# aerius-labs/paillier-halo2

Measured on AMD Instinct MI355X. Metric: Paillier-encrypt proofs/s (2048-bit n, k=17); MSM achieved HBM GB/s vs peak, higher is better.
Workload: dtype u32 limbs (29-bit reduced radix, 254-bit modular integers), u64 limbs (4096-bit integers)

## Files before the change

paillier_halo2_amd/csrc/pz_quotient.hip:

```cpp
#include "fp29.cuh"
#include "pz_internal.h"

static inline Fr fp_one_host() {
    static const uint64_t ONE[4] = {0xac96341c4ffffffbULL, 0x36fc76959f60cd29ULL, 0x666ea36f7879462eULL, 0x0e0a77c19a07df2fULL};
    Fr r;
    memcpy(r.v, ONE, 32);
    return r;
}
static inline Fr fr_from_u64(const uint64_t x[4]) {
    Fr r;
    memcpy(r.v, x, 32);
    return r;
}

typedef F29<FrTag> Fr29;
__device__ __forceinline__ Fr29 fr29_c261(const Fr& c) { return f29_to_261(f29_from_fp(c)); }
__device__ __forceinline__ Fr29 fr29_one256() {
    Fr29 r;
#pragma unroll
    for (int i = 0; i < 9; ++i) r.v[i] = P29<FrTag>::R256(i);
    return r;
}

struct S29 {
// ... 2 lines not shown
static bool host_fr_canonical(const uint64_t c[4]) {
    static const uint64_t R[4] = {0x43e1f593f0000001ULL, 0x2833e84879b97091ULL, 0xb85045b68181585dULL, 0x30644e72e131a029ULL};
    for (int i = 3; i >= 0; --i)
        if (c[i] != R[i]) return c[i] < R[i];
    return false;
}
static S29 host_fr_shl(const uint64_t c[4], unsigned k) {
    static const uint64_t R[4] = {0x43e1f593f0000001ULL, 0x2833e84879b97091ULL, 0xb85045b68181585dULL, 0x30644e72e131a029ULL};
    uint64_t x[4] = {c[0], c[1], c[2], c[3]};
    for (unsigned t = 0; t < k; ++t) {
        for (int i = 3; i > 0; --i) x[i] = (x[i] << 1) | (x[i - 1] >> 63);
        x[0] <<= 1;
        bool ge = true;
        for (int i = 3; i >= 0; --i)
            if (x[i] != R[i]) { ge = x[i] > R[i]; break; }
        if (ge) {
            unsigned __int128 br = 0;
            for (int i = 0; i < 4; ++i) {
                const unsigned __int128 d = (unsigned __int128)x[i] - R[i] - br;
                x[i] = (uint64_t)d;
                br = (d >> 64) & 1;
            }
        }
    }
    S29 r;
    for (int i = 0; i < 9; ++i) {
        const unsigned bit = 29u * i, j = bit >> 6, o = bit & 63;
        uint64_t w = x[j] >> o;
        if (o > 35 && j + 1 < 4) w |= x[j + 1] << (64 - o);
        r.v[i] = (u32)(w & (i < 8 ? 0x1fffffffull : 0xffffffffull));
    }
    return r;
}
static void host_fr_mul(const uint64_t a[4], const uint64_t b[4], uint64_t out[4]) {
    static const uint64_t R[4] = {0x43e1f593f0000001ULL, 0x2833e84879b97091ULL, 0xb85045b68181585dULL, 0x30644e72e131a029ULL};
    const uint64_t INV = 0xc2e1f593efffffffULL;
    uint64_t t[6] = {0, 0, 0, 0, 0, 0};
    for (int i = 0; i < 4; ++i) {
        unsigned __int128 c = 0;
        for (int j = 0; j < 4; ++j) {
            c += (unsigned __int128)a[j] * b[i] + t[j];
            t[j] = (uint64_t)c;
            c >>= 64;
        }
        c += t[4];
        t[4] = (uint64_t)c;
        t[5] = (uint64_t)(c >> 64);
        const uint64_t m = t[0] * INV;
        c = ((unsigned __int128)m * R[0] + t[0]) >> 64;
        for (int j = 1; j < 4; ++j) {
            c += (unsigned __int128)m * R[j] + t[j];
            t[j - 1] = (uint64_t)c;
            c >>= 64;
        }
        c += t[4];
        t[3] = (uint64_t)c;
        t[4] = t[5] + (uint64_t)(c >> 64);
    }
    bool ge = t[4] != 0;
    if (!ge) {
        ge = true;
        for (int i = 3; i >= 0; --i)
            if (t[i] != R[i]) { ge = t[i] > R[i]; break; }
    }
    if (ge) {
        unsigned __int128 br = 0;
// ... 170 lines not shown
    for (unsigned j = 0; j < PP_K && lo + j < n; ++j) {
        const Fr v = fp_load<FrTag>(a + lo + j);
        f29_store_product(z + lo + j, cur);
        cur = f29_mul(cur, f29_from_fp_shl5(v));
    }
}

int pz_prefix_product_batch_internal(pz_ctx* ctx, const Fr* d_a, size_t a_stride, size_t n_cols, size_t n, Fr z0, Fr* d_z,
                                     size_t z_stride) {
    if (!n || !n_cols) return PZ_OK;
    if (n_cols > 65535) return PZ_ERR_INVALID;
    const unsigned nb = pz_div_up(pz_div_up(n, PP_K), 256);
    void* ws;
    PZCHK(pz_ws_get(ctx, WS_BIG_B, n_cols * ((size_t)nb * 256 + nb) * 32, &ws));
    Fr* excl = (Fr*)ws;
    Fr* tot = excl + n_cols * (size_t)nb * 256;
    hipLaunchKernelGGL(k_pp_local, dim3(nb, (unsigned)n_cols), dim3(256), 0, ctx->stream, d_a, a_stride, n, excl, tot, nb);
    hipLaunchKernelGGL(k_pp_blocks, dim3(pz_div_up(n_cols, 64)), dim3(64), 0, ctx->stream, tot, nb, n_cols, z0);
    hipLaunchKernelGGL(k_pp_apply, dim3(nb, (unsigned)n_cols), dim3(256), 0, ctx->stream, d_a, a_stride, n, (const Fr*)excl,
                       (const Fr*)tot, nb, d_z, z_stride);
    HIPCHK(ctx, hipGetLastError());
    return PZ_OK;
}
int pz_prefix_product_internal(pz_ctx* ctx, const Fr* d_a, size_t n, Fr z0, Fr* d_z) {
    return pz_prefix_product_batch_internal(ctx, d_a, n, 1, n, z0, d_z, n);
}

extern "C" int pz_fr_prefix_product_dev(pz_ctx* ctx, const uint64_t* d_a, size_t n, const uint64_t z0[4], uint64_t* d_z) {
    if (!ctx || !z0 || (n && (!d_a || !d_z))) return PZ_ERR_INVALID;
    PZ_ENTER(ctx);
    return pz_prefix_product_internal(ctx, (const Fr*)d_a, n, fr_from_u64(z0), (Fr*)d_z);
}

__global__ __launch_bounds__(256) void k_perm_terms(const Fr* __restrict__ cols, size_t cs, const Fr* __restrict__ sigma,
                                                    size_t ss, unsigned m, size_t n, const Fr* __restrict__ wpow, Fr beta,
                                                    Fr gamma, Fr delta0, Fr delta, Fr* __restrict__ num,
                                                    Fr* __restrict__ den) {
    const size_t i = (size_t)blockIdx.x * blockDim.x + threadIdx.x;
    if (i >= n) return;
    const Fr29 g = fr29_c261(gamma), d = fr29_c261(delta), beta266 = f29_to_261(fr29_c261(beta));
    Fr29 nm = fr29_one256(), dn = nm;
    Fr29 bd = f29_mul(f29_mul(beta266, f29_from_fp(delta0)), f29_load_shl5<FrTag>(wpow + i));
    for (unsigned j = 0; j < m; ++j) {
        const Fr29 v = f29_add(f29_load_shl5<FrTag>(cols + (size_t)j * cs + i), g);
        const Fr29 sg = f29_load<FrTag>(sigma + (size_t)j * ss + i);
        nm = f29_mul(nm, f29_add(v, bd));
        dn = f29_mul(dn, f29_add(v, f29_mul(beta266, sg)));
        bd = f29_mul(bd, d);
    }
    f29_store<0>(num + i, nm);
    f29_store<0>(den + i, dn);
}

extern "C" int pz_permutation_product_dev(pz_ctx* ctx, const uint64_t* d_cols, size_t col_stride, const uint64_t* d_sigma,
                                          size_t sigma_stride, size_t m, uint32_t log_n, const uint64_t omega[4],
                                          const uint64_t beta[4], const uint64_t gamma[4], const uint64_t delta_start[4],
                                          const uint64_t delta[4], const uint64_t z0[4], uint64_t* d_z) {
    if (!ctx || !omega || !beta || !gamma || !delta_start || !delta || !z0 || !d_z || log_n > 26) return PZ_ERR_INVALID;
    if (m && (!d_cols || !d_sigma)) return PZ_ERR_INVALID;
    if (col_stride % 4 || sigma_stride % 4 || m > 65535) return PZ_ERR_INVALID;
    const size_t n = (size_t)1 << log_n;
    if (m > 1 && (col_stride < 4 * n || sigma_stride < 4 * n)) return PZ_ERR_INVALID;
    PZ_ENTER(ctx);
    void *wp, *ws;
    PZCHK(pz_get_pow_table(ctx, omega, n, &wp));
    PZCHK(pz_ws_get(ctx, WS_BIG_C, 2 * n * 32, &ws));
    Fr* num = (Fr*)ws;
    Fr* den = num + n;
    hipLaunchKernelGGL(k_perm_terms, dim3(pz_div_up(n, 256)), dim3(256), 0, ctx->stream, (const Fr*)d_cols, col_stride / 4,
                       (const Fr*)d_sigma, sigma_stride / 4, (unsigned)m, n, (const Fr*)wp, fr_from_u64(beta), fr_from_u64(gamma),
                       fr_from_u64(delta_start), fr_from_u64(delta), num, den);
    HIPCHK(ctx, hipGetLastError());
    PZCHK(pz_batch_invert_internal(ctx, den, n, num));
    return pz_prefix_product_internal(ctx, num, n, fr_from_u64(z0), (Fr*)d_z);
}

__global__ __launch_bounds__(256) void k_perm_terms_sets(const Fr* __restrict__ cols, size_t cs, const Fr* __restrict__ sigma,
                                                         size_t ss, unsigned m, unsigned chunk_len, size_t n,
                                                         const Fr* __restrict__ wpow, const Fr* __restrict__ dpow,
                                                         S29 beta266, S29 g, S29 d, Fr* __restrict__ num, Fr* __restrict__ den,
                                                         unsigned set0) {
    const size_t i = (size_t)blockIdx.x * blockDim.x + threadIdx.x;
    if (i >= n) return;
    const unsigned c0 = (set0 + blockIdx.y) * chunk_len, set = blockIdx.y;
    Fr29 nm = fr29_one256(), dn = nm;
    Fr29 bd = f29_mul(f29_mul_s(f29_load<FrTag>(dpow + c0), beta266.v), f29_load_shl5<FrTag>(wpow + i));
    Fr v_n = fp_load<FrTag>(cols + (size_t)c0 * cs + i), s_n = fp_load<FrTag>(sigma + (size_t)c0 * ss + i);
    for (unsigned c = c0; c < c0 + chunk_len && c < m; ++c) {
        const Fr29 v = f29_add_s(f29_from_fp_shl5(v_n), g.v);
        const Fr29 sg = f29_from_fp(s_n);
        const unsigned cn = (c + 1 < c0 + chunk_len && c + 1 < m) ? c + 1 : c;
        v_n = fp_load<FrTag>(cols + (size_t)cn * cs + i);
        s_n = fp_load<FrTag>(sigma + (size_t)cn * ss + i);
        nm = f29_mul(nm, f29_add(v, bd));
        dn = f29_mul(dn, f29_add(v, f29_mul_s(sg, beta266.v)));
        bd = f29_mul_s(bd, d.v);
    }
    f29_store_product(num + (size_t)set * n + i, nm);
// ... 15 lines not shown
            s_p[threadIdx.x] = p;
        }
        __syncthreads();
    }
    Fr c = threadIdx.x ? s_p[threadIdx.x - 1] : fp_one<FrTag>();
    for (unsigned j = lo; j < hi; ++j) {
        fp_store(mult + j, c);
        c = fp_mul(c, fp_load<FrTag>(z + (size_t)j * zs + u));
    }
}
__global__ __launch_bounds__(256) void k_scale_sets(Fr* __restrict__ z, size_t zs, size_t n, const Fr* __restrict__ mult) {
    const size_t i = (size_t)blockIdx.x * blockDim.x + threadIdx.x;
    if (i >= n || blockIdx.y == 0) return;
    Fr* p = z + (size_t)blockIdx.y * zs + i;
    fp_store(p, fp_mul(fp_load<FrTag>(p), fp_load<FrTag>(mult + blockIdx.y)));
}

extern "C" int pz_permutation_product_sets_dev(pz_ctx* ctx, const uint64_t* d_cols, size_t col_stride, const uint64_t* d_sigma,
                                               size_t sigma_stride, size_t m, uint32_t chunk_len, uint32_t log_n,
                                               size_t usable_rows, const uint64_t omega[4], const uint64_t beta[4],
                                               const uint64_t gamma[4], const uint64_t delta[4], uint64_t* d_z,
                                               size_t z_stride) {
    if (!ctx || !d_cols || !d_sigma || !d_z || !omega || !beta || !gamma || !delta || m == 0 || chunk_len == 0 || log_n > 26)
        return PZ_ERR_INVALID;
    const size_t n = (size_t)1 << log_n;
    const size_t n_sets = (m + chunk_len - 1) / chunk_len;
    if (col_stride % 4 || sigma_stride % 4 || z_stride % 4 || usable_rows >= n || n_sets > 65535 || m > 0xffffffu) return PZ_ERR_INVALID;
    if ((m > 1 && (col_stride < 4 * n || sigma_stride < 4 * n)) || (n_sets > 1 && z_stride < 4 * n)) return PZ_ERR_INVALID;
    if (!host_fr_canonical(beta) || !host_fr_canonical(gamma) || !host_fr_canonical(delta)) return PZ_ERR_INVALID;
    PZ_ENTER(ctx);
    void *wp, *dp, *ws, *mu;
    PZCHK(pz_get_pow_table(ctx, omega, n, &wp));
    PZCHK(pz_get_pow_table(ctx, delta, m, &dp));
    size_t sb = ((size_t)4 << 30) / (2 * n * 32);
    if (sb < 1) sb = 1;
    if (sb > n_sets) sb = n_sets;
    PZCHK(pz_ws_get(ctx, WS_BIG_C, 2 * sb * n * 32, &ws));
    PZCHK(pz_ws_get(ctx, WS_MISC, n_sets * 32, &mu));
    Fr* num = (Fr*)ws;
    Fr* den = num + sb * n;
    for (size_t s0 = 0; s0 < n_sets; s0 += sb) {
        const size_t ns = n_sets - s0 < sb ? n_sets - s0 : sb;
        hipLaunchKernelGGL(k_perm_terms_sets, dim3(pz_div_up(n, 256), (unsigned)ns), dim3(256), 0, ctx->stream,
                           (const Fr*)d_cols, col_stride / 4, (const Fr*)d_sigma, sigma_stride / 4, (unsigned)m, (unsigned)chunk_len, n,
                           (const Fr*)wp, (const Fr*)dp, host_fr_shl(beta, 10), host_fr_shl(gamma, 5), host_fr_shl(delta, 5), num, den,
                           (unsigned)s0);
        HIPCHK(ctx, hipGetLastError());
        PZCHK(pz_batch_invert_internal(ctx, den, ns * n, num));
        PZCHK(pz_prefix_product_batch_internal(ctx, num, n, ns, n, fp_one_host(), (Fr*)d_z + s0 * (z_stride / 4), z_stride / 4));
    }
    if (n_sets > 1) {
        hipLaunchKernelGGL(k_perm_chain, dim3(1), dim3(256), 0, ctx->stream, (const Fr*)d_z, z_stride / 4, (unsigned)n_sets,
                           usable_rows, (Fr*)mu);
        hipLaunchKernelGGL(k_scale_sets, dim3(pz_div_up(n, 256), (unsigned)n_sets), dim3(256), 0, ctx->stream, (Fr*)d_z,
                           z_stride / 4, n, (const Fr*)mu);
        HIPCHK(ctx, hipGetLastError());
    }
    return PZ_OK;
}

__global__ __launch_bounds__(256) void k_quotient_gate(const Fr* __restrict__ adv, size_t as, const Fr* __restrict__ sel,
                                                       size_t ss, unsigned n_cols, size_t N, unsigned step, S29 y261,
                                                       Fr* __restrict__ h) {
    const size_t i = (size_t)blockIdx.x * blockDim.x + threadIdx.x;
    if (i >= N) return;
    const size_t i1 = (i + step) & (N - 1), i2 = (i + 2 * (size_t)step) & (N - 1), i3 = (i + 3 * (size_t)step) & (N - 1);
// ... 387 lines not shown
```

paillier_halo2_amd/csrc/pz_msm.hip:

```cpp
#include "ec.cuh"
#include "ec29.cuh"
#include "ec29_quad.cuh"
#include <math.h>
#include <stdlib.h>

#include "pz_internal.h"

#define MSM_CHUNK_MIN 16u
#define MSM_CHUNK_MAX 256u
#define MSM_HEAVY 24u
#define MSM_MEDIUM 1024u
#define MSM_SLICE_MAX_COLS 8u

struct MsmP {
    size_t n;
    size_t n_table;
    unsigned c;
    unsigned nwin;
    unsigned win_lo, win_hi;
    unsigned B;
    size_t cap;
    size_t max_items;
    unsigned chunk;
    unsigned spt;
// ... 45 lines not shown
    u64 both = ((u64)hi << 32) | lo;
    unsigned raw = (unsigned)(both >> sh) & ((1u << c) - 1);
    unsigned d = raw + carry;
    if (d > (1u << (c - 1))) {
        carry = 1;
        return (int)d - (int)(1u << c);
    }
    carry = 0;
    return (int)d;
}

__global__ __launch_bounds__(128) void k_build_table(const G1Aff64* __restrict__ bases, G1Aff64* __restrict__ table,
                                                     size_t n, unsigned c, unsigned nwin) {
    size_t i = (size_t)blockIdx.x * blockDim.x + threadIdx.x;
    if (i >= n) return;
    G1A29 p = a29_load64(bases + i);
    if (!a29_is_inf(p)) {
        p.x = f29_to_261(p.x);
        p.y = f29_to_261(p.y);
        p = a29_canon(p);
    }
    a29_store64(table + i, p);
    G1X29 x = x29_from_affine(p);
    for (unsigned w = 1; w < nwin; ++w) {
        for (unsigned k = 0; k < c; ++k) x = x29_dbl(x);
        const G1A29 a = a29_canon(x29_to_affine(x));
        a29_store64(table + (size_t)w * n + i, a);
        x = x29_from_affine(a);
    }
}

#define SORT_THREADS 1024u
#ifndef SORT_PER_THREAD
#define SORT_PER_THREAD 8u
#endif
#define SORT_SLICE (SORT_THREADS * SORT_PER_THREAD)
#define SORT_MAXB 32768u

#ifndef PZ_SORT_XCD
#define PZ_SORT_XCD 1
#endif
__device__ __forceinline__ bool sort_block_coords(unsigned n_slices, size_t n_cols, unsigned& slice, size_t& col) {
    if (PZ_SORT_XCD && n_cols >= 8) {
        const unsigned w = blockIdx.x >> 3;
        slice = w % n_slices;
        col = (size_t)(w / n_slices) * 8 + (blockIdx.x & 7u);
    } else {
        slice = blockIdx.x % n_slices;
        col = blockIdx.x / n_slices;
    }
    return col < n_cols;
}
static unsigned sort_grid(unsigned n_slices, size_t n_cols) {
    if (PZ_SORT_XCD && n_cols >= 8) return n_slices * (unsigned)((n_cols + 7) / 8 * 8);
    return n_slices * (unsigned)n_cols;
}

__global__ __launch_bounds__(SORT_THREADS) void k_msm_hist(const Fr* __restrict__ scalars, size_t col_stride, MsmP p,
                                                           u32* __restrict__ slice_hist, unsigned n_slices, size_t n_cols) {
    __shared__ u32 h[SORT_MAXB];
    size_t col;
    unsigned slice;
    if (!sort_block_coords(n_slices, n_cols, slice, col)) return;
    for (unsigned b = threadIdx.x; b < p.B; b += SORT_THREADS) h[b] = 0;
    __syncthreads();
    const size_t base = (size_t)slice * SORT_THREADS * p.spt;
    for (unsigned t = 0; t < p.spt; ++t) {
// ... 781 lines not shown
            __syncthreads();
        }
        __syncthreads();
    }
}

struct alignas(16) MsmNode {
    G1X29Raw V, S;
};

__global__ __launch_bounds__(128) void k_msm_reduce_l1(MsmP p, unsigned m, const u32* __restrict__ items,
                                                       const G1X29Raw* __restrict__ partials, MsmNode* __restrict__ nodes) {
    const size_t col = blockIdx.y;
    const unsigned t = blockIdx.x * blockDim.x + threadIdx.x;
    const unsigned nn = p.B / m;
    if (t >= nn) return;
    const u32* it = items + col * (p.B + 1);
    const G1X29Raw* pc = partials + col * p.max_items;
    G1X29 run = x29_inf(), acc = x29_inf();
    for (unsigned j = m; j-- > 0;) {
        unsigned b = t * m + j;
        u32 a = it[b], z = it[b + 1];
        if (z > a) {
            G1X29 v = x29_load_raw(pc + a);
            x29_add(run, v);
        }
        x29_add(acc, run);
    }
    MsmNode* o = nodes + col * nn + t;
    x29_store_raw(&o->V, acc);
    x29_store_raw(&o->S, run);
}

__global__ __launch_bounds__(256) void k_msm_combine_quad(unsigned n_in, unsigned m, unsigned log_w,
                                                          const MsmNode* __restrict__ in, MsmNode* __restrict__ out) {
    const size_t col = blockIdx.y;
    const unsigned t = (blockIdx.x * blockDim.x + threadIdx.x) >> 2;
    const unsigned n_out = n_in / m;
    if (t >= n_out) return;
    const MsmNode* c = in + col * n_in + (size_t)t * m;
    G1X29 run = x29_inf(), acc = x29_inf();
    for (unsigned k = m; k-- > 1;) {
        const G1X29 s = x29_load_raw(&c[k].S);
        x29_add_quad(run, s);
        x29_add_quad(acc, run);
    }
    for (unsigned k = 0; k < log_w; ++k) acc = x29_dbl_quad(acc);
    const G1X29 s0 = x29_load_raw(&c[0].S);
    x29_add_quad(run, s0);
    for (unsigned k = 0; k < m; ++k) {
        const G1X29 v = x29_load_raw(&c[k].V);
        x29_add_quad(acc, v);
    }
    if ((threadIdx.x & 3u) == 0) {
        MsmNode* o = out + col * n_out + t;
        x29_store_raw(&o->V, acc);
        x29_store_raw(&o->S, run);
    }
}

__device__ __forceinline__ void lds_tree_sum_quad(G1X29Raw* s_pt, unsigned n) {
    const unsigned quad = threadIdx.x >> 2;
    for (unsigned off = n >> 1; off > 0; off >>= 1) {
        __syncthreads();
        for (unsigned node = quad; node < off; node += 64) {
            G1X29 a = x29_load_raw(&s_pt[node]);
            const G1X29 o = x29_load_raw(&s_pt[node + off]);
            x29_add_quad(a, o);
            if ((threadIdx.x & 3u) == 0) x29_store_raw(&s_pt[node], a);
        }
    }
    __syncthreads();
}

#define SLICE_SLOTS 9u
__global__ __launch_bounds__(256) void k_msm_slice_partial(MsmP p, const u32* __restrict__ items,
                                                           const G1X29Raw* __restrict__ partials, unsigned nblk,
                                                           G1X29Raw* __restrict__ slice_part) {
    __shared__ G1X29Raw s_pt[128];
    const size_t col = blockIdx.z;
    const unsigned y = blockIdx.y, blk = blockIdx.x;
    const u32* it = items + col * (p.B + 1);
    if (threadIdx.x < 128) {
        const unsigned i = threadIdx.x, yy = y < 8 ? y : 7u;
        const unsigned t = ((i >> yy) << (yy + 1)) | (y < 8 ? (1u << yy) : 0u) | (i & ((1u << yy) - 1u));
        const unsigned w = blk * 256u + t;
        G1X29 v = x29_inf();
        if (w >= 1 && w <= p.B) {
            const u32 a = it[w - 1], z = it[w];
            if (z > a) v = x29_load_raw(partials + col * p.max_items + a);
// ... 183 lines not shown
    delete b;
    return PZ_OK;
}

extern "C" int pz_bases_info(const pz_bases* b, size_t* n_points, uint32_t* window_bits, uint32_t* n_windows) {
    if (!b) return PZ_ERR_INVALID;
    if (n_points) *n_points = b->n;
    if (window_bits) *window_bits = b->c;
    if (n_windows) *n_windows = b->nwin;
    return PZ_OK;
}

static unsigned msm_chunk_for(size_t n_cols, size_t digits_per_col, unsigned window_bits) {
    static int env = -1;
    if (env < 0) {
        const char* e = getenv("PZ_MSM_CHUNK");
        env = e ? atoi(e) : 0;
    }
    if (env >= (int)MSM_CHUNK_MIN && env <= (int)MSM_CHUNK_MAX) return (unsigned)env;
    if (n_cols <= MSM_SLICE_MAX_COLS) {
        const double per_bucket = (double)digits_per_col / (double)((size_t)1 << (window_bits - 1));
        double ch = 0.79 * pow(per_bucket, 0.63);
        unsigned c32 = ch < 24.0 ? MSM_CHUNK_MIN : 32u * (unsigned)((ch + 16.0) / 32.0);
        if (c32 > MSM_CHUNK_MAX) c32 = MSM_CHUNK_MAX;
        return c32;
    }
    const size_t want = (n_cols * digits_per_col) >> 18;
    unsigned chunk = MSM_CHUNK_MIN;
    while (chunk < MSM_CHUNK_MAX && chunk * 2 <= want) chunk *= 2;
    return chunk;
}

static unsigned msm_spt_for(size_t n_cols, size_t n) {
    const size_t min_wg = n_cols <= MSM_SLICE_MAX_COLS ? 128 : 512;
    unsigned spt = SORT_PER_THREAD;
    while (spt > 1 && n_cols * pz_div_up(n, (size_t)SORT_THREADS * spt) < min_wg) spt >>= 1;
    return spt;
}

static int msm_group(pz_ctx* ctx, const pz_bases* bases, const Fr* d_scalars, size_t nc, size_t n, size_t cs,
                     unsigned win_lo, unsigned win_hi, unsigned chunk, G1Jac* d_out) {
    MsmP p;
    p.n = n;
    p.n_table = bases->n;
    p.c = bases->c;
    p.nwin = bases->nwin;
    p.win_lo = win_lo;
    p.win_hi = win_hi;
    p.B = 1u << (bases->c - 1);
    p.cap = n * (size_t)(win_hi - win_lo);
    p.chunk = chunk;
    if (p.B + n * (size_t)(win_hi - win_lo) / chunk > 65535u * 256u) return PZ_ERR_CAPACITY;
    p.max_items = p.B + p.cap / chunk;
    void *hist, *offs, *heavy, *items, *entries, *partials, *na, *nb, *totals, *fold, *iord;
    p.spt = msm_spt_for(nc, n);
    const unsigned n_slices = pz_div_up(n, (size_t)SORT_THREADS * p.spt);
    PZCHK(pz_ws_get(ctx, WS_HIST, nc * (size_t)n_slices * p.B * 4, &hist));
    PZCHK(pz_ws_get(ctx, WS_CURSOR, nc * (size_t)(p.B + 1) * 4, &heavy));
    const bool split_items = nc <= MSM_SLICE_MAX_COLS;
    const unsigned nblk_few = pz_div_up(p.B, 256);
    PZCHK(pz_ws_get(ctx, WS_TOTALS, nc * ((size_t)p.B + (split_items ? (size_t)nblk_few * (2 + FEW_BINS) : 0)) * 4, &totals));
    u32* blk_cnt = (u32*)totals + nc * (size_t)p.B;
    u32* blk_itm = blk_cnt + nc * (size_t)nblk_few;
    u32* blk_bins = blk_itm + nc * (size_t)nblk_few;
    u32* heavy_cnt = (u32*)heavy + nc * (size_t)p.B;
    PZCHK(pz_ws_get(ctx, WS_MISC, nc * (size_t)(p.B + 1) * 4, &fold));
    u32* fold_cnt = (u32*)fold + nc * (size_t)p.B;
    PZCHK(pz_ws_get(ctx, WS_ORDER, nc * p.max_items * 8, &iord));
    u32* item_order = (u32*)iord;
    u32* item_bucket = (u32*)iord + nc * p.max_items;
    PZCHK(pz_ws_get(ctx, WS_OFFS, nc * (p.B + 1) * 4, &offs));
    PZCHK(pz_ws_get(ctx, WS_ITEMS, nc * (p.B + 1) * 4, &items));
    PZCHK(pz_ws_get(ctx, WS_ENTRIES, nc * p.cap * 4 + 16, &entries));
    static int scatter_mode = -1;
    if (scatter_mode < 0) {
        const char* e = getenv("PZ_MSM_SCATTER");
        scatter_mode = (e && !strcmp(e, "one")) ? 1 : (e && !strcmp(e, "two")) ? 2 : 0;
    }
    const bool two_pass = scatter_mode != 1 && p.c == 16 && (size_t)p.nwin * p.n_table <= ((size_t)1 << 24) &&
                          (nc > MSM_SLICE_MAX_COLS || scatter_mode == 2);
    {
        const size_t part_bytes = nc * p.max_items * sizeof(G1X29Raw), stage_bytes = two_pass ? nc * p.cap * 4 + 16 : 0;
        PZCHK(pz_ws_get(ctx, WS_PARTIALS, part_bytes > stage_bytes ? part_bytes : stage_bytes, &partials));
    }
    const unsigned m1 = p.B >= 16 ? 16 : p.B;
    unsigned n_nodes = p.B / m1;
    PZCHK(pz_ws_get(ctx, WS_NODES_A, nc * (size_t)n_nodes * sizeof(MsmNode), &na));
    PZCHK(pz_ws_get(ctx, WS_NODES_B, nc * (size_t)(n_nodes / 2 + 1) * sizeof(MsmNode), &nb));
    hipStream_t st = ctx->stream;
    pz_timer tall(ctx, PZ_T_MSM_ALL);
    dim3 gs(sort_grid(n_slices, nc));
    void* dsel;
    PZCHK(pz_ws_get(ctx, WS_SEL, 8, &dsel));
    HIPCHK(ctx, hipMemsetAsync(dsel, 0, 8, st));
    PZCHK(pz_async_err_init(ctx));
    {
        pz_timer tsort(ctx, PZ_T_MSM_SORT);
        hipLaunchKernelGGL(k_msm_hist, gs, dim3(SORT_THREADS), 0, st, d_scalars, cs, p, (u32*)hist, n_slices, nc);
        if (split_items) {
            hipLaunchKernelGGL(k_msm_totals_few, dim3(nblk_few, (unsigned)nc), dim3(256), 0, st, (u32*)hist, n_slices, p, (u32*)totals,
                               blk_cnt, blk_itm, blk_bins);
            hipLaunchKernelGGL(k_msm_items_few, dim3(nblk_few, (unsigned)nc), dim3(256), 0, st, p, (const u32*)totals, (const u32*)blk_cnt,
                               (const u32*)blk_itm, (const u32*)blk_bins, (u32*)offs, (u32*)items, item_order, item_bucket,
                               (unsigned long long*)dsel);
        } else {
            hipLaunchKernelGGL(k_msm_totals, dim3(pz_div_up(p.B, 256), (unsigned)nc), dim3(256), 0, st, (u32*)hist, n_slices, p,
                               (u32*)totals);
            hipLaunchKernelGGL(k_msm_scan, dim3((unsigned)nc), dim3(SCAN_THREADS), 0, st, (const u32*)totals, p, (u32*)offs, (u32*)items,
                               (u32*)heavy, heavy_cnt, (u32*)fold, fold_cnt, item_order, item_bucket, (unsigned long long*)dsel);
        }
        ScatterSel sel;
        sel.total = (const unsigned long long*)dsel;
        sel.thr = !two_pass ? ~0ull : scatter_mode == 2 ? 0ull : (unsigned long long)(0.4 * (double)nc * (double)p.cap);
        sel.err = ctx->async_err_d;
        if (two_pass) {
            hipLaunchKernelGGL(k_msm_scatter_coarse, gs, dim3(COARSE_THREADS), 0, st, d_scalars, cs, p, (const u32*)hist, n_slices,
                               (const u32*)offs, (u32*)partials, nc, sel);
            hipLaunchKernelGGL(k_msm_scatter_fine, dim3(p.B >> SORT_FINE_LOG, (unsigned)nc), dim3(FINE_THREADS), 0, st, p, (const u32*)offs,
                               (const u32*)partials, (u32*)entries, sel);
        }
        if (scatter_mode != 2 || !two_pass)
// ... 9 lines not shown
    pz_timer ttree(ctx, PZ_T_MSM_TREE);
    if (split_items) {
        const unsigned gx4 = pz_div_up(p.B, 64), gx32 = p.B / 8 < 2048u ? (p.B / 8 ? p.B / 8 : 1u) : 2048u;
        hipLaunchKernelGGL(k_msm_fold_few, dim3(gx4, (unsigned)nc), dim3(256), 0, st, p, (const u32*)items, (G1X29Raw*)partials, 2u, 1u, MSM_FEW_SMALL);
        hipLaunchKernelGGL(k_msm_fold_few, dim3(gx32, (unsigned)nc), dim3(256), 0, st, p, (const u32*)items, (G1X29Raw*)partials, 5u, MSM_FEW_SMALL,
                           MSM_MEDIUM);
        hipLaunchKernelGGL(k_msm_heavy_few, dim3(p.B / 256 < 64u ? (p.B / 256 ? p.B / 256 : 1u) : 64u, (unsigned)nc), dim3(256), 0, st, p,
                           (const u32*)items, (G1X29Raw*)partials);
    } else {
    hipLaunchKernelGGL(k_msm_bucket_sum, dim3((unsigned)nc, pz_div_up(p.B, 256)), dim3(256), 0, st, p, (const u32*)items,
                       (const u32*)fold, (const u32*)fold_cnt, (G1X29Raw*)partials);
    unsigned hx = (unsigned)(8192 / nc);
    if (hx < 4) hx = 4;
    if (hx > p.B) hx = p.B;
    hipLaunchKernelGGL(k_msm_heavy_sum, dim3(hx, (unsigned)nc), dim3(256), 0, st, p, (const u32*)items, (const u32*)heavy,
                       (const u32*)heavy_cnt, (G1X29Raw*)partials);
    hipLaunchKernelGGL(k_msm_medium_sum, dim3(hx, (unsigned)nc), dim3(256), 0, st, p, (const u32*)items, (const u32*)heavy,
                       (const u32*)heavy_cnt, (G1X29Raw*)partials);
    }
    if (nc <= MSM_SLICE_MAX_COLS) {
        const unsigned nblk = (p.B >> 8) + 1;
        void *sp, *sl;
        PZCHK(pz_ws_get(ctx, WS_NODES_A, nc * (size_t)SLICE_SLOTS * nblk * sizeof(G1X29Raw), &sp));
        PZCHK(pz_ws_get(ctx, WS_NODES_B, nc * 16 * sizeof(G1X29Raw), &sl));
        hipLaunchKernelGGL(k_msm_slice_partial, dim3(nblk, SLICE_SLOTS, (unsigned)nc), dim3(256), 0, st, p, (const u32*)items,
                           (const G1X29Raw*)partials, nblk, (G1X29Raw*)sp);
        hipLaunchKernelGGL(k_msm_slice_reduce, dim3(p.c, (unsigned)nc), dim3(256), 0, st, p, nblk, (const G1X29Raw*)sp, (G1X29Raw*)sl);
        hipLaunchKernelGGL(k_msm_slice_horner, dim3((unsigned)nc), dim3(64), 0, st, p, (const G1X29Raw*)sl, d_out);
        HIPCHK(ctx, hipGetLastError());
        return PZ_OK;
    }
    hipLaunchKernelGGL(k_msm_reduce_l1, dim3(pz_div_up(n_nodes, 128), (unsigned)nc), dim3(128), 0, st, p, m1,
                       (const u32*)items, (const G1X29Raw*)partials, (MsmNode*)na);
    const unsigned m1_used = m1;
    MsmNode* cur = (MsmNode*)na;
    MsmNode* nxt = (MsmNode*)nb;
    unsigned log_w = 0;
    for (unsigned t = m1_used; t > 1; t >>= 1) ++log_w;
    while (n_nodes > 1) {
        unsigned m = n_nodes >= 16 ? 16 : n_nodes;
        hipLaunchKernelGGL(k_msm_combine_quad, dim3(pz_div_up((size_t)(n_nodes / m) * 4, 256), (unsigned)nc), dim3(256), 0, st, n_nodes, m,
                           log_w, (const MsmNode*)cur, nxt);
        n_nodes /= m;
        for (unsigned t = m; t > 1; t >>= 1) ++log_w;
        MsmNode* tmp = cur;
        cur = nxt;
        nxt = tmp;
    }
    hipLaunchKernelGGL(k_msm_emit, dim3(pz_div_up(nc, 64)), dim3(64), 0, st, (const MsmNode*)cur, nc, d_out);
    HIPCHK(ctx, hipGetLastError());
    return PZ_OK;
}

extern "C" int pz_msm_g1_dev(pz_ctx* ctx, const pz_bases* bases, const uint64_t* d_scalars, size_t n_cols, size_t n,
                             size_t col_stride, uint32_t win_lo, uint32_t win_hi, uint64_t* d_out_jac) {
    if (!ctx || !bases || (n_cols && (!d_scalars || !d_out_jac))) return PZ_ERR_INVALID;
    if (n > bases->n || win_lo > win_hi || win_hi > bases->nwin) return PZ_ERR_INVALID;
    if (col_stride % 4 || (n_cols > 1 && col_stride < 4 * n)) return PZ_ERR_INVALID;
    if (n_cols == 0) return PZ_OK;
    PZ_ENTER(ctx);
    if (n == 0 || win_lo == win_hi) {
        size_t nn = n_cols;
        void* z;
        PZCHK(pz_ws_get(ctx, WS_NODES_A, nn * sizeof(MsmNode), &z));
        HIPCHK(ctx, hipMemsetAsync(z, 0, nn * sizeof(MsmNode), ctx->stream));
        hipLaunchKernelGGL(k_msm_emit, dim3(pz_div_up(nn, 64)), dim3(64), 0, ctx->stream, (const MsmNode*)z, nn,
                           (G1Jac*)d_out_jac);
        HIPCHK(ctx, hipGetLastError());
        return PZ_OK;
    }
    const size_t cs = col_stride / 4;
    const size_t digits = n * (size_t)(win_hi - win_lo);
    const unsigned chunk = msm_chunk_for(n_cols, digits, bases->c);
    const size_t part_col = (digits / chunk) * sizeof(G1X29Raw);
    const size_t per_col = digits * 4 + (part_col > digits * 4 ? part_col : digits * 4) + (digits / chunk) * 8 +
                           (size_t)(1u << (bases->c - 1)) * (180 + 4 * (size_t)pz_div_up(n, (size_t)SORT_THREADS * msm_spt_for(1, n)));
    size_t ws_budget = pz_msm_ws_gib() << 30;
    {
        if (ctx->mem_avail == 0 || ++ctx->mem_avail_age >= 64) {
            const size_t free_b = pz_mem_free_bytes(ctx);
            if (free_b) {
                size_t held = 0;
// ... 283 lines not shown
```

Measured before the change: 1.290.

## Fuse permutation product terms, batch inversion and prefix product into segmented passes

Replaces the separate passes (compute num/den terms, batch-invert den, prefix-product num) with a fused pipeline. One kernel computes the terms, writes den and the running numerator prefix, and does per-segment forward and backward products in shared memory. A small segment kernel performs the single inversion per set, a chain kernel carries products across sets, and an apply kernel walks each run backward to combine the inverse and prefix. This removes a full num array and several HBM round trips and kernel launches. In exchange it adds segment tables, a serial per-set segment loop, a single-block chain, and more complex code. The old path stays behind an environment variable.

```diff
diff --git a/paillier_halo2_amd/csrc/pz_quotient.hip b/paillier_halo2_amd/csrc/pz_quotient.hip
--- a/paillier_halo2_amd/csrc/pz_quotient.hip
+++ b/paillier_halo2_amd/csrc/pz_quotient.hip
@@ -58,6 +58,18 @@
     }
     return r;
 }
+static void host_fr_reduce(const uint64_t c[4], uint64_t out[4]) {
+    static const uint64_t R[4] = {0x43e1f593f0000001ULL, 0x2833e84879b97091ULL, 0xb85045b68181585dULL, 0x30644e72e131a029ULL};
+    memcpy(out, c, 32);
+    while (!host_fr_canonical(out)) {
+        unsigned __int128 br = 0;
+        for (int i = 0; i < 4; ++i) {
+            const unsigned __int128 d = (unsigned __int128)out[i] - R[i] - br;
+            out[i] = (uint64_t)d;
+            br = (d >> 64) & 1;
+        }
+    }
+}
 static void host_fr_mul(const uint64_t a[4], const uint64_t b[4], uint64_t out[4]) {
     static const uint64_t R[4] = {0x43e1f593f0000001ULL, 0x2833e84879b97091ULL, 0xb85045b68181585dULL, 0x30644e72e131a029ULL};
     const uint64_t INV = 0xc2e1f593efffffffULL;
@@ -294,6 +306,208 @@
     return pz_prefix_product_internal(ctx, (const Fr*)d_a, n, fr_from_u64(z0), (Fr*)d_z);
 }
 
+#define PF_RUN 16u
+#define PF_SEG (256u * PF_RUN)
+__device__ __forceinline__ Fr29 f29_shl5_strict(const Fr29& a) {
+    Fr29 r;
+    r.v[0] = (a.v[0] << 5) & F29_MASK;
+#pragma unroll
+    for (int i = 1; i < 8; ++i) r.v[i] = ((a.v[i] << 5) & F29_MASK) | (a.v[i - 1] >> 24);
+    r.v[8] = (a.v[8] << 5) | (a.v[7] >> 24);
+    return r;
+}
+__global__ __launch_bounds__(256) void k_pf_terms(const Fr* __restrict__ cols, size_t cs, const Fr* __restrict__ sigma, size_t ss,
+                                                  unsigned m, unsigned chunk_len, size_t n, size_t u, const Fr* __restrict__ wpow,
+                                                  const Fr* __restrict__ dpow, S29 beta266, S29 g, S29 d, S29 bd0,
+                                                  Fr* __restrict__ z, size_t zs, Fr* __restrict__ den, Fr* __restrict__ kt,
+                                                  Fr* __restrict__ segt, Fr* __restrict__ xu, unsigned set0) {
+    __shared__ u32 s_n[9 * 256], s_d[9 * 256];
+    const unsigned t = threadIdx.x, set = blockIdx.y, n_seg = gridDim.x;
+    const unsigned c0 = (set0 + set) * chunk_len;
+    const size_t lo = (size_t)blockIdx.x * PF_SEG + (size_t)t * PF_RUN, hi = lo + PF_RUN < n ? lo + PF_RUN : n;
+    const bool own_u = u >= lo && u < hi;
+    z += (size_t)set * zs;
+    den += (size_t)set * n;
+    Fr29 rn = fr29_one256(), rd = rn, su = rn, pu = rn;
+    for (size_t i = lo; i < hi; ++i) {
+        Fr29 nm = fr29_one256(), dn = nm;
+        const Fr29 w5 = f29_load_shl5<FrTag>(wpow + i);
+        Fr29 bd = dpow ? f29_mul(f29_mul_s(f29_load<FrTag>(dpow + c0), beta266.v), w5) : f29_mul_s(w5, bd0.v);
+        if (c0 < m) {
+            Fr v_n = fp_load<FrTag>(cols + (size_t)c0 * cs + i), s_n1 = fp_load<FrTag>(sigma + (size_t)c0 * ss + i);
+            for (unsigned c = c0; c < c0 + chunk_len && c < m; ++c) {
+                const Fr29 v = f29_add_s(f29_from_fp_shl5(v_n), g.v);
+                const Fr29 sg = f29_from_fp(s_n1);
+                const unsigned cn = (c + 1 < c0 + chunk_len && c + 1 < m) ? c + 1 : c;
+                v_n = fp_load<FrTag>(cols + (size_t)cn * cs + i);
+                s_n1 = fp_load<FrTag>(sigma + (size_t)cn * ss + i);
+                nm = f29_mul(nm, f29_add(v, bd));
+                dn = f29_mul(dn, f29_add(v, f29_mul_s(sg, beta266.v)));
+                bd = f29_mul_s(bd, d.v);
+            }
+        }
+        if (f29_is_zero(dn)) {
+            nm = f29_zero<FrTag>();
+            dn = fr29_one256();
+        }
+        f29_store_product(den + i, dn);
+        f29_store_product(z + i, rn);
+        if (i == u) pu = rn;
+        rn = f29_mul(rn, f29_shl5_strict(nm));
+        const Fr29 d5 = f29_shl5_strict(dn);
+        rd = f29_mul(rd, d5);
+        if (own_u && i >= u) su = f29_mul(su, d5);
+    }
+    Fr29 fn = f29_to_261(rn), bk = f29_to_261(rd);
+#pragma unroll
+    for (int i = 0; i < 9; ++i) {
+        s_n[i * 256 + t] = fn.v[i];
+        s_d[i * 256 + t] = bk.v[i];
+    }
+    __syncthreads();
+    for (unsigned off = 1; off < 256; off <<= 1) {
+        Fr29 a, b;
+        if (t >= off) {
+#pragma unroll
+            for (int i = 0; i < 9; ++i) a.v[i] = s_n[i * 256 + t - off];
+        }
+        if (t + off < 256) {
+#pragma unroll
+            for (int i = 0; i < 9; ++i) b.v[i] = s_d[i * 256 + t + off];
+        }
+        __syncthreads();
+        if (t >= off) {
+            fn = f29_mul(a, fn);
+#pragma unroll
+            for (int i = 0; i < 9; ++i) s_n[i * 256 + t] = fn.v[i];
+        }
+        if (t + off < 256) {
+            bk = f29_mul(b, bk);
+#pragma unroll
+            for (int i = 0; i < 9; ++i) s_d[i * 256 + t] = bk.v[i];
+        }
+        __syncthreads();
+    }
+    Fr29 before = f29_one<FrTag>(), after = f29_one<FrTag>();
+    if (t) {
+#pragma unroll
+        for (int i = 0; i < 9; ++i) before.v[i] = s_n[i * 256 + t - 1];
+    }
+    if (t < 255) {
+#pragma unroll
+        for (int i = 0; i < 9; ++i) after.v[i] = s_d[i * 256 + t + 1];
+    }
+    const Fr29 k261 = f29_mul(before, after);
+    const size_t sg_idx = (size_t)set * n_seg + blockIdx.x;
+    {
+        Fr w;
+        f29_pack(k261, w.v);
+        fp_store(kt + sg_idx * 256 + t, w);
+    }
+    if (t == 255) f29_store_product(segt + 2 * sg_idx, f29_to_256(fn));
+    if (t == 0) f29_store_product(segt + 2 * sg_idx + 1, f29_to_256(bk));
+    if (own_u) f29_store_product(xu + set, f29_mul(f29_mul(k261, pu), f29_shl5_strict(su)));
+}
+__global__ __launch_bounds__(64) void k_pf_segments(Fr* __restrict__ segt, unsigned n_seg, Fr* __restrict__ xu, size_t ns,
+                                                    unsigned seg_u) {
+    const size_t j = (size_t)blockIdx.x * blockDim.x + threadIdx.x;
+    if (j >= ns) return;
+    Fr* p = segt + j * n_seg * 2;
+    Fr pn = fp_one<FrTag>(), pd = pn;
+    for (unsigned s = 0; s < n_seg; ++s) {
+        const Fr a = fp_load<FrTag>(p + 2 * s), b = fp_load<FrTag>(p + 2 * s + 1);
+        fp_store(p + 2 * s, pn);
+        pn = fp_mul(pn, a);
+        pd = fp_mul(pd, b);
+    }
+    Fr inv = fp_inv(pd);
+    for (unsigned s = n_seg; s-- > 0;) {
+        fp_store(p + 2 * s, fp_mul(fp_load<FrTag>(p + 2 * s), inv));
+        inv = fp_mul(inv, fp_load<FrTag>(p + 2 * s + 1));
+    }
+    fp_store(xu + j, fp_mul(fp_load<FrTag>(p + 2 * seg_u), fp_load<FrTag>(xu + j)));
+}
+__global__ __launch_bounds__(256) void k_pf_chain(Fr* __restrict__ zu, unsigned ns, Fr* __restrict__ carry, Fr init, int first) {
+    __shared__ Fr s_p[256];
+    const unsigned per = (ns + 255u) / 256u, lo = threadIdx.x * per, hi = lo + per < ns ? lo + per : ns;
+    const Fr c_in = first ? init : fp_load<FrTag>(carry);
+    Fr p = fp_one<FrTag>();
+    for (unsigned j = lo; j < hi; ++j) p = fp_mul(p, fp_load<FrTag>(zu + j));
+    s_p[threadIdx.x] = p;
+    __syncthreads();
+    for (unsigned off = 1; off < 256; off <<= 1) {
+        Fr v = fp_one<FrTag>();
+        if (threadIdx.x >= off) v = s_p[threadIdx.x - off];
+        __syncthreads();
+        if (threadIdx.x >= off) {
+            p = fp_mul(v, p);
+            s_p[threadIdx.x] = p;
+        }
+        __syncthreads();
+    }
+    Fr c = threadIdx.x ? fp_mul(c_in, s_p[threadIdx.x - 1]) : c_in;
+    for (unsigned j = lo; j < hi; ++j) {
+        const Fr v = fp_load<FrTag>(zu + j);
+        fp_store(zu + j, c);
+        c = fp_mul(c, v);
+    }
+    if (lo < hi && hi == ns) fp_store(carry, c);
+}
+__global__ __launch_bounds__(256) void k_pf_apply(Fr* __restrict__ z, size_t zs, const Fr* __restrict__ den, size_t n,
+                                                  const Fr* __restrict__ kt, const Fr* __restrict__ segt, const Fr* __restrict__ mult) {
+    const unsigned t = threadIdx.x, set = blockIdx.y;
+    const size_t lo = (size_t)blockIdx.x * PF_SEG + (size_t)t * PF_RUN;
+    if (lo >= n) return;
+    const size_t hi = lo + PF_RUN < n ? lo + PF_RUN : n, sg_idx = (size_t)set * gridDim.x + blockIdx.x;
+    z += (size_t)set * zs;
+    den += (size_t)set * n;
+    Fr29 acc = f29_mul(f29_load<FrTag>(segt + 2 * sg_idx), f29_load_shl5<FrTag>(mult + set));
+    acc = f29_mul(acc, f29_load<FrTag>(kt + sg_idx * 256 + t));
+    for (size_t i = hi; i-- > lo;) {
+        acc = f29_mul(acc, f29_load_shl5<FrTag>(den + i));
+        f29_store_product(z + i, f29_mul(acc, f29_load_shl5<FrTag>(z + i)));
+    }
+}
+
+static bool pz_perm_passes() {
+    static int mode = -1;
+    if (mode < 0) {
+        const char* e = getenv("PZ_PERM_PRODUCT");
+        mode = (e && !strcmp(e, "passes")) ? 1 : 0;
+    }
+    return mode == 1;
+}
+
+static int pz_perm_product_fused(pz_ctx* ctx, const Fr* cols, size_t cs, const Fr* sigma, size_t ss, unsigned m, unsigned chunk_len,
+                                 size_t n_sets, size_t n, size_t u, const Fr* wp, const Fr* dp, S29 beta266, S29 g, S29 d, S29 bd0,
+                                 Fr z0, Fr* z, size_t zs) {
+    const unsigned n_seg = pz_div_up(n, PF_SEG);
+    size_t sb = ((size_t)2 << 30) / (n * 32);
+    if (sb < 1) sb = 1;
+    if (sb > n_sets) sb = n_sets;
+    const size_t per_set = n + (size_t)n_seg * 256 + (size_t)n_seg * 2 + 1;
+    void* ws;
+    PZCHK(pz_ws_get(ctx, WS_BIG_C, (sb * per_set + 1) * 32, &ws));
+    Fr* den = (Fr*)ws;
+    Fr* kt = den + sb * n;
+    Fr* segt = kt + sb * n_seg * 256;
+    Fr* xu = segt + sb * n_seg * 2;
+    Fr* carry = xu + sb;
+    for (size_t s0 = 0; s0 < n_sets; s0 += sb) {
+        const size_t ns = n_sets - s0 < sb ? n_sets - s0 : sb;
+        Fr* zb = z + s0 * zs;
+        hipLaunchKernelGGL(k_pf_terms, dim3(n_seg, (unsigned)ns), dim3(256), 0, ctx->stream, cols, cs, sigma, ss, m, chunk_len, n, u, wp,
+                           dp, beta266, g, d, bd0, zb, zs, den, kt, segt, xu, (unsigned)s0);
+        hipLaunchKernelGGL(k_pf_segments, dim3(pz_div_up(ns, 64)), dim3(64), 0, ctx->stream, segt, n_seg, xu, ns,
+                           (unsigned)(u / PF_SEG));
+        hipLaunchKernelGGL(k_pf_chain, dim3(1), dim3(256), 0, ctx->stream, xu, (unsigned)ns, carry, z0, (int)(s0 == 0));
+        hipLaunchKernelGGL(k_pf_apply, dim3(n_seg, (unsigned)ns), dim3(256), 0, ctx->stream, zb, zs, (const Fr*)den, n, (const Fr*)kt,
+                           (const Fr*)segt, (const Fr*)xu);
+        HIPCHK(ctx, hipGetLastError());
+    }
+    return PZ_OK;
+}
+
 __global__ __launch_bounds__(256) void k_perm_terms(const Fr* __restrict__ cols, size_t cs, const Fr* __restrict__ sigma,
                                                     size_t ss, unsigned m, size_t n, const Fr* __restrict__ wpow, Fr beta,
                                                     Fr gamma, Fr delta0, Fr delta, Fr* __restrict__ num,
@@ -326,6 +540,17 @@
     PZ_ENTER(ctx);
     void *wp, *ws;
     PZCHK(pz_get_pow_table(ctx, omega, n, &wp));
+    if (!pz_perm_passes()) {
+        uint64_t b[4], g[4], d0[4], d[4], bd0[4];
+        host_fr_reduce(beta, b);
+        host_fr_reduce(gamma, g);
+        host_fr_reduce(delta_start, d0);
+        host_fr_reduce(delta, d);
+        host_fr_mul(b, d0, bd0);
+        return pz_perm_product_fused(ctx, (const Fr*)d_cols, col_stride / 4, (const Fr*)d_sigma, sigma_stride / 4, (unsigned)m,
+                                     (unsigned)m, 1, n, 0, (const Fr*)wp, nullptr, host_fr_shl(b, 10), host_fr_shl(g, 5),
+                                     host_fr_shl(d, 5), host_fr_shl(bd0, 5), fr_from_u64(z0), (Fr*)d_z, n);
+    }
     PZCHK(pz_ws_get(ctx, WS_BIG_C, 2 * n * 32, &ws));
     Fr* num = (Fr*)ws;
     Fr* den = num + n;
@@ -407,6 +632,10 @@
     void *wp, *dp, *ws, *mu;
     PZCHK(pz_get_pow_table(ctx, omega, n, &wp));
     PZCHK(pz_get_pow_table(ctx, delta, m, &dp));
+    if (!pz_perm_passes())
+        return pz_perm_product_fused(ctx, (const Fr*)d_cols, col_stride / 4, (const Fr*)d_sigma, sigma_stride / 4, (unsigned)m,
+                                     chunk_len, n_sets, n, usable_rows, (const Fr*)wp, (const Fr*)dp, host_fr_shl(beta, 10),
+                                     host_fr_shl(gamma, 5), host_fr_shl(delta, 5), S29{}, fp_one_host(), (Fr*)d_z, z_stride / 4);
     size_t sb = ((size_t)4 << 30) / (2 * n * 32);
     if (sb < 1) sb = 1;
     if (sb > n_sets) sb = n_sets;
```

New measurement: 1.301 (median of 6 runs). Within noise of the previous version (+0.9%).

## Fuse MSM bucket-reduction tail into one kernel and raise sort items per thread

Applied to the files above, without the earlier changes.

Once 128 or fewer nodes remain per column, the final combine levels and the emit step run in a single block-per-column kernel that keeps intermediates in shared memory, replacing several tiny launches. The default sort items per thread rises from 8 to 32 for many-column MSMs, while few-column MSMs stay capped at 8, and a PZ_MSM_SPT override is added. The secondary node buffer shrinks because the first combine level now always divides by 16. The tail kernel uses only one 64-thread block per column, which may serialize work when many columns are present, and the larger per-thread sort slice changes sort occupancy.

```diff
diff --git a/paillier_halo2_amd/csrc/pz_msm.hip b/paillier_halo2_amd/csrc/pz_msm.hip
--- a/paillier_halo2_amd/csrc/pz_msm.hip
+++ b/paillier_halo2_amd/csrc/pz_msm.hip
@@ -101,7 +101,7 @@
 
 #define SORT_THREADS 1024u
 #ifndef SORT_PER_THREAD
-#define SORT_PER_THREAD 8u
+#define SORT_PER_THREAD 32u
 #endif
 #define SORT_SLICE (SORT_THREADS * SORT_PER_THREAD)
 #define SORT_MAXB 32768u
@@ -949,30 +949,66 @@
     x29_store_raw(&o->S, run);
 }
 
+__device__ __forceinline__ void combine_node_quad(const MsmNode* c, unsigned m, unsigned log_w, G1X29& acc, G1X29& run) {
+    run = x29_inf();
+    acc = x29_inf();
+    for (unsigned k = m; k-- > 1;) {
+        const G1X29 s = x29_load_raw(&c[k].S);
+        x29_add_quad(run, s);
+        x29_add_quad(acc, run);
+    }
+    for (unsigned k = 0; k < log_w; ++k) acc = x29_dbl_quad(acc);
+    const G1X29 s0 = x29_load_raw(&c[0].S);
+    x29_add_quad(run, s0);
+    for (unsigned k = 0; k < m; ++k) {
+        const G1X29 v = x29_load_raw(&c[k].V);
+        x29_add_quad(acc, v);
+    }
+}
 __global__ __launch_bounds__(256) void k_msm_combine_quad(unsigned n_in, unsigned m, unsigned log_w,
                                                           const MsmNode* __restrict__ in, MsmNode* __restrict__ out) {
     const size_t col = blockIdx.y;
     const unsigned t = (blockIdx.x * blockDim.x + threadIdx.x) >> 2;
     const unsigned n_out = n_in / m;
     if (t >= n_out) return;
-    const MsmNode* c = in + col * n_in + (size_t)t * m;
-    G1X29 run = x29_inf(), acc = x29_inf();
-    for (unsigned k = m; k-- > 1;) {
-        const G1X29 s = x29_load_raw(&c[k].S);
-        x29_add_quad(run, s);
-        x29_add_quad(acc, run);
-    }
-    for (unsigned k = 0; k < log_w; ++k) acc = x29_dbl_quad(acc);
-    const G1X29 s0 = x29_load_raw(&c[0].S);
-    x29_add_quad(run, s0);
-    for (unsigned k = 0; k < m; ++k) {
-        const G1X29 v = x29_load_raw(&c[k].V);
-        x29_add_quad(acc, v);
-    }
+    G1X29 acc, run;
+    combine_node_quad(in + col * n_in + (size_t)t * m, m, log_w, acc, run);
     if ((threadIdx.x & 3u) == 0) {
         MsmNode* o = out + col * n_out + t;
         x29_store_raw(&o->V, acc);
         x29_store_raw(&o->S, run);
+    }
+}
+
+#define TAIL_MAX_IN 128u
+#define TAIL_THREADS 64u
+__global__ __launch_bounds__(TAIL_THREADS) void k_msm_combine_tail(unsigned n_in, unsigned log_w, const MsmNode* __restrict__ in,
+                                                                   G1Jac* __restrict__ out) {
+    __shared__ MsmNode s_n[TAIL_THREADS / 4];
+    const size_t col = blockIdx.x;
+    const unsigned q = threadIdx.x >> 2;
+    const MsmNode* src = in + col * n_in;
+    if (n_in == 1) {
+        if (threadIdx.x == 0) x29_store_jac(out + col, x29_load_raw(&src[0].V));
+        return;
+    }
+    while (n_in > 1) {
+        const unsigned m = n_in >= 16 ? 16 : n_in, n_out = n_in / m;
+        G1X29 acc, run;
+        if (q < n_out) combine_node_quad(src + (size_t)q * m, m, log_w, acc, run);
+        __syncthreads();
+        if (q < n_out && (threadIdx.x & 3u) == 0) {
+            if (n_out == 1) {
+                x29_store_jac(out + col, acc);
+            } else {
+                x29_store_raw(&s_n[q].V, acc);
+                x29_store_raw(&s_n[q].S, run);
+            }
+        }
+        __syncthreads();
+        n_in = n_out;
+        for (unsigned t = m; t > 1; t >>= 1) ++log_w;
+        src = s_n;
     }
 }
 
@@ -1222,8 +1258,14 @@
 }
 
 static unsigned msm_spt_for(size_t n_cols, size_t n) {
+    static int env = -1;
+    if (env < 0) {
+        const char* e = getenv("PZ_MSM_SPT");
+        env = e ? atoi(e) : 0;
+    }
     const size_t min_wg = n_cols <= MSM_SLICE_MAX_COLS ? 128 : 512;
-    unsigned spt = SORT_PER_THREAD;
+    unsigned spt = n_cols <= MSM_SLICE_MAX_COLS ? (SORT_PER_THREAD < 8u ? SORT_PER_THREAD : 8u) : SORT_PER_THREAD;
+    while (env > 0 && spt > 1 && spt > (unsigned)env) spt >>= 1;
     while (spt > 1 && n_cols * pz_div_up(n, (size_t)SORT_THREADS * spt) < min_wg) spt >>= 1;
     return spt;
 }
@@ -1276,7 +1318,7 @@
     const unsigned m1 = p.B >= 16 ? 16 : p.B;
     unsigned n_nodes = p.B / m1;
     PZCHK(pz_ws_get(ctx, WS_NODES_A, nc * (size_t)n_nodes * sizeof(MsmNode), &na));
-    PZCHK(pz_ws_get(ctx, WS_NODES_B, nc * (size_t)(n_nodes / 2 + 1) * sizeof(MsmNode), &nb));
+    PZCHK(pz_ws_get(ctx, WS_NODES_B, nc * (size_t)(n_nodes / 16 + 1) * sizeof(MsmNode), &nb));
     hipStream_t st = ctx->stream;
     pz_timer tall(ctx, PZ_T_MSM_ALL);
     dim3 gs(sort_grid(n_slices, nc));
@@ -1352,22 +1394,21 @@
     }
     hipLaunchKernelGGL(k_msm_reduce_l1, dim3(pz_div_up(n_nodes, 128), (unsigned)nc), dim3(128), 0, st, p, m1,
                        (const u32*)items, (const G1X29Raw*)partials, (MsmNode*)na);
-    const unsigned m1_used = m1;
     MsmNode* cur = (MsmNode*)na;
     MsmNode* nxt = (MsmNode*)nb;
     unsigned log_w = 0;
-    for (unsigned t = m1_used; t > 1; t >>= 1) ++log_w;
-    while (n_nodes > 1) {
-        unsigned m = n_nodes >= 16 ? 16 : n_nodes;
+    for (unsigned t = m1; t > 1; t >>= 1) ++log_w;
+    while (n_nodes > TAIL_MAX_IN) {
+        const unsigned m = 16;
         hipLaunchKernelGGL(k_msm_combine_quad, dim3(pz_div_up((size_t)(n_nodes / m) * 4, 256), (unsigned)nc), dim3(256), 0, st, n_nodes, m,
                            log_w, (const MsmNode*)cur, nxt);
         n_nodes /= m;
-        for (unsigned t = m; t > 1; t >>= 1) ++log_w;
+        log_w += 4;
         MsmNode* tmp = cur;
         cur = nxt;
         nxt = tmp;
     }
-    hipLaunchKernelGGL(k_msm_emit, dim3(pz_div_up(nc, 64)), dim3(64), 0, st, (const MsmNode*)cur, nc, d_out);
+    hipLaunchKernelGGL(k_msm_combine_tail, dim3((unsigned)nc), dim3(TAIL_THREADS), 0, st, n_nodes, log_w, (const MsmNode*)cur, d_out);
     HIPCHK(ctx, hipGetLastError());
     return PZ_OK;
 }
diff --git a/profiles/msm_overhead_split.py b/profiles/msm_overhead_split.py
--- /dev/null
+++ b/profiles/msm_overhead_split.py
@@ -0,0 +1,54 @@
+import collections
+import csv
+import sys
+
+
+def _short(name):
+    return name.split("(")[0].replace("void ", "").strip()
+
+
+def split(path):
+    rows = []
+    with open(path, newline="") as f:
+        for r in csv.DictReader(f):
+            name = r.get("Kernel_Name") or r.get("KernelName") or r.get("Name") or ""
+            if "k_msm_" not in name:
+                continue
+            t0, t1 = int(r["Start_Timestamp"]), int(r["End_Timestamp"])
+            rows.append((t0, t1 - t0, _short(name)))
+    rows.sort()
+    seqs, cur = [], None
+    for t0, d, k in rows:
+        if k == "k_msm_hist":
+            cur = collections.defaultdict(int)
+            seqs.append(cur)
+        if cur is not None:
+            cur[k] += d
+    kinds = collections.OrderedDict((k, collections.defaultdict(int)) for k in ("dense", "sparse", "few"))
+    count = collections.Counter()
+    for s in seqs:
+        kind = "few" if "k_msm_totals_few" in s else "dense" if s["k_msm_scatter_coarse"] > s["k_msm_scatter"] else "sparse"
+        count[kind] += 1
+        for k, v in s.items():
+            kinds[kind][k] += v
+    return kinds, count
+
+
+def main(paths):
+    for p in paths:
+        kinds, count = split(p)
+        print("# %s" % p)
+        for kind, tot in kinds.items():
+            acc = tot.get("k_msm_accumulate", 0)
+            rest = sum(v for k, v in tot.items() if k != "k_msm_accumulate")
+            print("%-6s sequences %4d   accumulate %9.1f ms   outside it %9.1f ms" % (kind, count[kind], acc / 1e6, rest / 1e6))
+            for k, v in sorted(tot.items(), key=lambda kv: -kv[1]):
+                if k != "k_msm_accumulate":
+                    print("         %-24s %9.2f ms" % (k, v / 1e6))
+        allacc = sum(t.get("k_msm_accumulate", 0) for t in kinds.values())
+        allrest = sum(v for t in kinds.values() for k, v in t.items() if k != "k_msm_accumulate")
+        print("all    accumulate %9.1f ms   outside it %9.1f ms\n" % (allacc / 1e6, allrest / 1e6))
+
+
+if __name__ == "__main__":
+    main(sys.argv[1:])
```

Result: no change. 1.295 before, 1.308 after, median of 6 (+1.0%).
